# pymoc/pymoc

Measured on AMD Instinct MI355X. Metric: column-timesteps/sec (ensemble) at nz=100, higher is better.
Workload: dtype f64; 1 GPU; BASELINE configs[1]: 1024 independent Columns x nz=100 fp64 per GPU, static wA, do_conv on odd members, dt=30 d (pymoc_amd.configs.config2); columns_per_gpu=1024, nz=100, kernel=k_column_steps<64,2,6,true,true>, parallelism=ensemble sharded over 1 GPU(s), RCCL gather (root) of the final state

## Files before the change

### pymoc_amd/csrc/column.hip.h

```cpp
#pragma once
#include <type_traits>
#include "common.hip.h"

namespace pm {

template <int P>
struct ColGrid {
  double z[P];
  double dz[P];
  double dzc[P];
  double rdz[P], rdzc[P];
  double rdz_l[P], rdzc_l[P];
};
template <int P>
struct ColRegs {
  double b[P];
  double kap[P];
  double area[P];
  double dAk[P];
  double rarea[P];
  double rarea_l[P];
  double area_u, rarea_u, rarea_lu;
};

template <int P>
__device__ __forceinline__ void load_levels(double (&out)[P], const double *__restrict__ row,
                                            int lg, int nz, int lvl0 = 0) {
  if constexpr (P == 2) {
    if (lvl0 == 0 && (nz & 1) == 0 && (((unsigned long long)row) & 15ull) == 0ull) {
      const int i0 = lg * 2 < nz - 2 ? lg * 2 : nz - 2;
      const double2 v = *reinterpret_cast<const double2 *>(row + i0);
      out[0] = v.x;
      out[1] = v.y;
      return;
    }
  }
#pragma unroll
  for (int p = 0; p < P; ++p) {
    const int i = lvl0 + lg * P + p;
    out[p] = row[i < nz ? i : nz - 1];
  }
}

template <int P>
__device__ __forceinline__ double level_value(const double (&x)[P], int j) {
  const int jl = __builtin_amdgcn_readfirstlane(j / P);
  const int jp = __builtin_amdgcn_readfirstlane(j % P);
  double out = 0.;
#pragma unroll
  for (int p = 0; p < P; ++p) {
    const int lo = __builtin_amdgcn_readlane(__double2loint(x[p]), jl);
    const int hi = __builtin_amdgcn_readlane(__double2hiint(x[p]), jl);
    const double v = __hiloint2double(hi, lo);
    out = (p == 0 || jp == p) ? v : out;
  }
  return out;
}

__device__ __forceinline__ double lane_value(double x, int lane) {
  const int lo = __builtin_amdgcn_readlane(__double2loint(x), lane);
  const int hi = __builtin_amdgcn_readlane(__double2hiint(x), lane);
  return __hiloint2double(hi, lo);
}

template <int P>
struct ConvCache {
  unsigned long long mask[P];
  double zconv;
  bool valid = false;
};

template <int G, int P>
__device__ __forceinline__ bool col_convect(double (&b)[P], const double (&z)[P],
                                            double bs, double N2min, int lg, int lane,
                                            int nz, const double *__restrict__ zg,
                                            ConvCache<P> *cache = nullptr) {
  const unsigned long long gm = group_mask<G>(lane);
  bool ind[P];
  unsigned long long im[P];
  unsigned long long anym = 0ull;
#pragma unroll
  for (int p = 0; p < P; ++p) {
    const int i = lg * P + p;
    ind[p] = (i < nz) && (b[p] > bs);
    im[p] = __builtin_amdgcn_ballot_w64(ind[p]);
    anym |= im[p] & gm;
  }
  if (__builtin_expect(anym != 0ull, 0)) {
    double zconv;
    bool hit = false;
    if constexpr (G == 64) {
      if (cache != nullptr && cache->valid) {
        hit = true;
#pragma unroll
        for (int p = 0; p < P; ++p) hit = hit && (cache->mask[p] == im[p]);
      }
    }
    if (hit) {
      zconv = cache->zconv;
    } else {
      int jmax = 0;
#pragma unroll
      for (int p = 0; p < P; ++p) {
        const int i = lg * P + p;
        const unsigned long long m = __builtin_amdgcn_ballot_w64((i < nz) && !ind[p]) & gm;
        if (m != 0ull) {
          const int hl = 63 - __clzll((long long)m);
          const int j = (hl % G) * P + p;
          jmax = j > jmax ? j : jmax;
        }
      }
      if constexpr (G == 64) {
        zconv = level_value<P>(z, jmax);
        if (cache != nullptr) {
#pragma unroll
          for (int p = 0; p < P; ++p) cache->mask[p] = im[p];
          cache->zconv = zconv;
          cache->valid = true;
        }
      } else {
        zconv = zg[jmax];
      }
    }
#pragma unroll
    for (int p = 0; p < P; ++p) {
      const double adj = bs + N2min * (z[p] - zconv);
      b[p] = ind[p] ? adj : b[p];
    }
    return true;
  }
#pragma unroll
  for (int p = 0; p < P; ++p)
    if (lg * P + p == nz - 1) b[p] = bs;
  return false;
}

template <int P>
__device__ __forceinline__ void col_convect_cached(double (&b)[P], const double (&z)[P],
                                                   double bs, double N2min, int lane, int nz,
                                                   ConvCache<P> &cc) {
  bool ind[P];
  unsigned long long im[P], anym = 0ull;
  bool same = cc.valid;
#pragma unroll
  for (int p = 0; p < P; ++p) {
    ind[p] = (lane * P + p < nz) && (b[p] > bs);
    im[p] = __builtin_amdgcn_ballot_w64(ind[p]);
    anym |= im[p];
    same = same && (im[p] == cc.mask[p]);
  }
  if (__builtin_expect(!same, 0)) {
    int jmax = 0;
#pragma unroll
    for (int p = 0; p < P; ++p) {
      const unsigned long long m = __builtin_amdgcn_ballot_w64((lane * P + p < nz) && !ind[p]);
      if (m != 0ull) {
        const int j = (63 - __clzll((long long)m)) * P + p;
        jmax = j > jmax ? j : jmax;
      }
    }
    cc.zconv = level_value<P>(z, jmax);
#pragma unroll
    for (int p = 0; p < P; ++p) cc.mask[p] = im[p];
    cc.valid = true;
  }
  const bool none = anym == 0ull;
#pragma unroll
  for (int p = 0; p < P; ++p) {
    const double adj = bs + N2min * (z[p] - cc.zconv);
    b[p] = ind[p] ? adj : b[p];
    if (lane * P + p == nz - 1) b[p] = none ? bs : b[p];
  }
}

template <int G, int P, int DIV, bool BC = true, bool WEFF = false, bool UA = false,
          bool FLUXFMA = (DIV == 2 || DIV >= 6)>
__device__ __forceinline__ void col_vertadvdiff(const ColGrid<P> &g, ColRegs<P> &r,
                                                const double (&wA)[P],
                                                double dt, bool do_conv, double bs,
                                                double bbot, bool use_bzbot,
                                                double bzbot, int lg, int nz,
                                                int lvl0 = 0) {
  if (BC && !do_conv) {
#pragma unroll
    for (int p = 0; p < P; ++p)
      if (lvl0 + lg * P + p == nz - 1) r.b[p] = bs;
  }
  const double nb0 = from_next_lane_z(r.b[0]);
  double bup[P];
#pragma unroll
  for (int p = 0; p < P; ++p) bup[p] = (p < P - 1) ? r.b[p + 1 < P ? p + 1 : p] : nb0;
  if (BC && lvl0 + lg * P == 0) r.b[0] = use_bzbot ? (bup[0] - bzbot * g.dz[0]) : bbot;

  if constexpr (DIV == 4) {
    double d_up[P];
#pragma unroll
    for (int p = 0; p < P; ++p) d_up[p] = bup[p] - r.b[p];
    const double pd = from_prev_lane_z(d_up[P - 1]);
#pragma unroll
    for (int p = 0; p < P; ++p) {
      const double d_dn = (p > 0) ? d_up[p > 0 ? p - 1 : 0] : pd;
      r.b[p] = __builtin_fma(r.kap[p], d_up[p], __builtin_fma(r.dAk[p], d_dn, r.b[p]));
    }
    return;
  }
  double bz[P];
  {
    double num[P], q[P], rr[P];
#pragma unroll
    for (int p = 0; p < P; ++p) num[p] = bup[p] - r.b[p];
    if constexpr (DIV == 2) {
#pragma unroll
      for (int p = 0; p < P; ++p) rr[p] = num[p] * g.rdz_l[p];
#pragma unroll
      for (int p = 0; p < P; ++p) q[p] = __builtin_fma(num[p], g.rdz[p], rr[p]);
#pragma unroll
      for (int p = 0; p < P; ++p) rr[p] = __builtin_fma(-g.dz[p], q[p], num[p]);
#pragma unroll
      for (int p = 0; p < P; ++p) q[p] = __builtin_fma(rr[p], g.rdz[p], q[p]);
    } else if constexpr (DIV == 7 || DIV == 8) {
#pragma unroll
      for (int p = 0; p < P; ++p) rr[p] = num[p] * g.rdz_l[p];
#pragma unroll
      for (int p = 0; p < P; ++p) q[p] = __builtin_fma(num[p], g.rdz[p], rr[p]);
    } else if constexpr (DIV == 6) {
#pragma unroll
      for (int p = 0; p < P; ++p) q[p] = num[p] * g.rdz[p];
#pragma unroll
      for (int p = 0; p < P; ++p) rr[p] = __builtin_fma(-g.dz[p], q[p], num[p]);
#pragma unroll
      for (int p = 0; p < P; ++p) q[p] = __builtin_fma(rr[p], g.rdz[p], q[p]);
    } else if constexpr (DIV == 1 || DIV == 3 || DIV == 5) {
#pragma unroll
      for (int p = 0; p < P; ++p) q[p] = num[p] * g.rdz[p];
#pragma unroll
      for (int p = 0; p < P; ++p) rr[p] = __builtin_fma(-g.dz[p], q[p], num[p]);
#pragma unroll
      for (int p = 0; p < P; ++p) q[p] = __builtin_fma(rr[p], g.rdz[p], q[p]);
#pragma unroll
      for (int p = 0; p < P; ++p) rr[p] = __builtin_fma(-g.dz[p], q[p], num[p]);
#pragma unroll
      for (int p = 0; p < P; ++p) q[p] = __builtin_fma(rr[p], g.rdz[p], q[p]);
    } else {
#pragma unroll
      for (int p = 0; p < P; ++p) q[p] = num[p] / g.dz[p];
    }
    if constexpr (DIV != 0) {
#pragma unroll
      for (int p = 0; p < P; ++p) bz[p] = q[p];
    } else {
#pragma unroll
      for (int p = 0; p < P; ++p) bz[p] = (lvl0 + lg * P + p < nz - 1) ? q[p] : 0.0;
    }
  }
  const double pbz = from_prev_lane_z(bz[P - 1]);
  double bz_dn[P], dbz[P], flx[P], bzz[P], adv[P];
#pragma unroll
  for (int p = 0; p < P; ++p) {
    bz_dn[p] = (p > 0) ? bz[p > 0 ? p - 1 : 0] : pbz;
    dbz[p] = bz[p] - bz_dn[p];
    const double weff = WEFF ? wA[p] : wA[p] - r.dAk[p];
    if constexpr (FLUXFMA) {
      const double wn = (weff < 0.0) ? -weff : 0.0, wp = (weff < 0.0) ? 0.0 : -weff;
      flx[p] = __builtin_fma(wn, bz[p], wp * bz_dn[p]);
    } else {
      const double bzu = (weff < 0.0) ? bz[p] : bz_dn[p];
      flx[p] = (-weff) * bzu;
    }
  }
  if constexpr (DIV == 2) {
    double r1[P], r2[P];
#pragma unroll
    for (int p = 0; p < P; ++p) {
      r1[p] = dbz[p] * g.rdzc_l[p];
      r2[p] = flx[p] * (UA ? r.rarea_lu : r.rarea_l[p]);
    }
#pragma unroll
    for (int p = 0; p < P; ++p) {
      bzz[p] = __builtin_fma(dbz[p], g.rdzc[p], r1[p]);
      adv[p] = __builtin_fma(flx[p], (UA ? r.rarea_u : r.rarea[p]), r2[p]);
    }
#pragma unroll
    for (int p = 0; p < P; ++p) {
      r1[p] = __builtin_fma(-g.dzc[p], bzz[p], dbz[p]);
      r2[p] = __builtin_fma(-(UA ? r.area_u : r.area[p]), adv[p], flx[p]);
    }
#pragma unroll
    for (int p = 0; p < P; ++p) {
      bzz[p] = __builtin_fma(r1[p], g.rdzc[p], bzz[p]);
      adv[p] = __builtin_fma(r2[p], (UA ? r.rarea_u : r.rarea[p]), adv[p]);
    }
  } else if constexpr (DIV == 6) {
    double r1[P], r2[P];
#pragma unroll
    for (int p = 0; p < P; ++p) {
      bzz[p] = dbz[p] * g.rdzc[p];
      adv[p] = flx[p] * (UA ? r.rarea_u : r.rarea[p]);
    }
#pragma unroll
    for (int p = 0; p < P; ++p) {
      r1[p] = __builtin_fma(-g.dzc[p], bzz[p], dbz[p]);
      r2[p] = __builtin_fma(-(UA ? r.area_u : r.area[p]), adv[p], flx[p]);
    }
#pragma unroll
    for (int p = 0; p < P; ++p) {
      bzz[p] = __builtin_fma(r1[p], g.rdzc[p], bzz[p]);
      adv[p] = __builtin_fma(r2[p], (UA ? r.rarea_u : r.rarea[p]), adv[p]);
    }
  } else if constexpr (DIV == 8) {
    double r1[P], r2[P];
#pragma unroll
    for (int p = 0; p < P; ++p) {
      r1[p] = dbz[p] * g.rdzc_l[p];
      r2[p] = flx[p] * (UA ? r.rarea_lu : r.rarea_l[p]);
    }
#pragma unroll
    for (int p = 0; p < P; ++p) {
      bzz[p] = __builtin_fma(dbz[p], g.rdzc[p], r1[p]);
      adv[p] = __builtin_fma(flx[p], (UA ? r.rarea_u : r.rarea[p]), r2[p]);
    }
  } else if constexpr (DIV == 7) {
    double r1[P], r2[P];
#pragma unroll
    for (int p = 0; p < P; ++p) {
      r1[p] = dbz[p] * g.rdzc_l[p];
      adv[p] = flx[p] * (UA ? r.rarea_u : r.rarea[p]);
    }
#pragma unroll
    for (int p = 0; p < P; ++p) {
      bzz[p] = __builtin_fma(dbz[p], g.rdzc[p], r1[p]);
      r2[p] = __builtin_fma(-(UA ? r.area_u : r.area[p]), adv[p], flx[p]);
    }
#pragma unroll
    for (int p = 0; p < P; ++p) adv[p] = __builtin_fma(r2[p], (UA ? r.rarea_u : r.rarea[p]), adv[p]);
  } else if constexpr (DIV == 5) {
    double r1[P];
#pragma unroll
    for (int p = 0; p < P; ++p) {
      bzz[p] = dbz[p] * g.rdzc[p];
      adv[p] = div_by_recip2(flx[p], r.area_u, r.rarea_u, r.rarea_lu);
    }
#pragma unroll
    for (int k = 0; k < 2; ++k) {
#pragma unroll
      for (int p = 0; p < P; ++p) r1[p] = __builtin_fma(-g.dzc[p], bzz[p], dbz[p]);
#pragma unroll
      for (int p = 0; p < P; ++p) bzz[p] = __builtin_fma(r1[p], g.rdzc[p], bzz[p]);
    }
  } else if constexpr (DIV == 3) {
    double r1[P];
#pragma unroll
    for (int p = 0; p < P; ++p) {
      bzz[p] = dbz[p] * g.rdzc[p];
      adv[p] = flx[p] / (UA ? r.area_u : r.area[p]);
    }
#pragma unroll
    for (int k = 0; k < 2; ++k) {
#pragma unroll
      for (int p = 0; p < P; ++p) r1[p] = __builtin_fma(-g.dzc[p], bzz[p], dbz[p]);
#pragma unroll
      for (int p = 0; p < P; ++p) bzz[p] = __builtin_fma(r1[p], g.rdzc[p], bzz[p]);
    }
  } else if constexpr (DIV == 1) {
    double r1[P], r2[P];
#pragma unroll
    for (int p = 0; p < P; ++p) {
      bzz[p] = dbz[p] * g.rdzc[p];
      adv[p] = flx[p] * (UA ? r.rarea_u : r.rarea[p]);
    }
#pragma unroll
    for (int k = 0; k < 2; ++k) {
#pragma unroll
      for (int p = 0; p < P; ++p) {
        r1[p] = __builtin_fma(-g.dzc[p], bzz[p], dbz[p]);
        r2[p] = __builtin_fma(-(UA ? r.area_u : r.area[p]), adv[p], flx[p]);
      }
#pragma unroll
      for (int p = 0; p < P; ++p) {
        bzz[p] = __builtin_fma(r1[p], g.rdzc[p], bzz[p]);
        adv[p] = __builtin_fma(r2[p], (UA ? r.rarea_u : r.rarea[p]), adv[p]);
      }
    }
  } else {
#pragma unroll
    for (int p = 0; p < P; ++p) {
      bzz[p] = dbz[p] / g.dzc[p];
      adv[p] = flx[p] / (UA ? r.area_u : r.area[p]);
    }
  }
#pragma unroll
  for (int p = 0; p < P; ++p) {
    const int i = lvl0 + lg * P + p;
    const bool interior = (i >= 1) && (i <= nz - 2);
    const double db_dt = adv[p] + r.kap[p] * bzz[p];
    if constexpr (DIV == 0) {
      const double nb = r.b[p] + dt * db_dt;
      r.b[p] = interior ? nb : r.b[p];
    } else {
      r.b[p] = r.b[p] + (interior ? dt : 0.0) * db_dt;
    }
  }
}

template <int P>
__device__ __forceinline__ void col_horadv(ColRegs<P> &r, const double (&vdx)[P],
                                           const double (&bin)[P], double dt, int lg,
                                           int nz) {
#pragma unroll
  for (int p = 0; p < P; ++p) {
    const int i = lg * P + p;
    if (i < nz && vdx[p] > 0.0) {
      const double db = bin[p] - r.b[p];
      r.b[p] = r.b[p] + dt * vdx[p] * db / r.area[p];
    }
  }
}

template <int P>
__device__ __forceinline__ bool col_inputs_in_fast_range(const ColGrid<P> &g, const ColRegs<P> &r,
                                                         const double (&wA)[P], double dt,
                                                         double bs, double bbot, double bzbot,
                                                         double N2min, int lg, int nz) {
  bool ok = in_fast_div_range(dt) && in_fast_div_range(bs) && in_fast_div_range(bbot) &&
            in_fast_div_range(bzbot) && in_fast_div_range(N2min);
#pragma unroll
  for (int p = 0; p < P; ++p) {
    const bool top = lg * P + p >= nz - 1;
    ok = ok && in_fast_div_range(r.b[p]) && in_fast_div_range(wA[p]) &&
         in_fast_div_range(r.dAk[p]) && in_fast_div_range(wA[p] - r.dAk[p]) &&
         in_fast_div_range(r.kap[p]) && in_fast_div_range(r.area[p]) && r.area[p] != 0.0 &&
         in_fast_div_range(g.z[p]) && (top || (in_fast_div_range(g.dz[p]) && g.dz[p] != 0.0)) &&
         in_fast_div_range(g.dzc[p]) && g.dzc[p] != 0.0;
  }
  return ok;
}

template <int P>
__device__ __forceinline__ bool col_state_in_fast_range(const ColRegs<P> &r, const double (&wA)[P]) {
  int ok = 1;
#pragma unroll
  for (int p = 0; p < P; ++p)
    ok &= (int)in_fast_div_range(r.b[p]) & (int)in_fast_div_range(wA[p] - r.dAk[p]);
  return ok != 0;
}

template <int P, int DIV = 1>
__device__ __forceinline__ void col_load_grid(ColGrid<P> &g, const pm_columns &c, int lg,
                                              int lvl0 = 0) {
  const int nz = c.nz;
#pragma unroll
  for (int p = 0; p < P; ++p) {
    const int i = lvl0 + lg * P + p;
    const int ic = i < nz ? i : nz - 1;
    const int iu = ic + 1 < nz ? ic + 1 : nz - 1;
    const int id = ic > 0 ? ic - 1 : 0;
    const double zc = c.z[ic];
    g.z[p] = zc;
    g.dz[p] = c.z[iu] - zc;
    g.dzc[p] = 0.5 * (g.dz[p] + (zc - c.z[id]));
    if constexpr (DIV != 0 && DIV != 4) {
      g.rdz[p] = (i < nz - 1) ? 1.0 / g.dz[p] : 0.0;
      g.rdzc[p] = 1.0 / g.dzc[p];
    } else {
      g.rdz[p] = g.rdzc[p] = 0.0;
    }
    if constexpr (DIV == 2) {
      g.rdz_l[p] = (i < nz - 1) ? recip_lo(g.dz[p], g.rdz[p]) : 0.0;
      g.rdzc_l[p] = recip_lo(g.dzc[p], g.rdzc[p]);
    } else {
      g.rdz_l[p] = g.rdzc_l[p] = 0.0;
    }
  }
}

template <int P, int DIV = 1>
__device__ __forceinline__ void col_load_static(ColRegs<P> &r, const pm_columns &c,
                                                int col, int sel, int lg, int lvl0 = 0,
                                                bool uniform_area = false, bool weff_in = false) {
  const int nz = c.nz;
  const size_t base = (size_t)col * nz;
  const size_t sbase = ((size_t)sel * c.ncols + col) * nz;
  load_levels<P>(r.kap, c.kappa + sbase, lg, nz, lvl0);
  if (!weff_in) {
    load_levels<P>(r.dAk, c.dAkappa + sbase, lg, nz, lvl0);
  } else {
#pragma unroll
    for (int p = 0; p < P; ++p) r.dAk[p] = 0.0;
  }
  if (uniform_area) {
    const double a0 = c.area[base];
    const double ra = (DIV != 0 && DIV != 4) ? 1.0 / a0 : 0.0;
    const double ral = DIV == 2 ? recip_lo(a0, ra) : 0.0;
#pragma unroll
    for (int p = 0; p < P; ++p) {
      r.area[p] = a0;
      r.rarea[p] = ra;
      r.rarea_l[p] = ral;
    }
    return;
  }
  load_levels<P>(r.area, c.area + base, lg, nz, lvl0);
#pragma unroll
  for (int p = 0; p < P; ++p) {
    r.rarea[p] = (DIV != 0 && DIV != 4) ? 1.0 / r.area[p] : 0.0;
    r.rarea_l[p] = DIV == 2 ? recip_lo(r.area[p], r.rarea[p]) : 0.0;
  }
}

template <int P>
__device__ __forceinline__ void col_make_contracted(const ColGrid<P> &g, ColRegs<P> &r,
                                                    const double (&wA)[P], double dt, int lane,
                                                    int nz) {
  const double dz_prev_lane = from_prev_lane_z(g.dz[P - 1]);
#pragma unroll
  for (int p = 0; p < P; ++p) {
    const int i = lane * P + p;
    const bool interior = i >= 1 && i <= nz - 2;
    const double weff = wA[p] - r.dAk[p];
    const double dz_up = interior ? g.dz[p] : 1.0;
    const double dz_dn = interior ? ((p > 0) ? g.dz[p > 0 ? p - 1 : 0] : dz_prev_lane) : 1.0;
    const double dzc = interior ? g.dzc[p] : 1.0, area = interior ? r.area[p] : 1.0;
    const double wn = (weff < 0.0) ? -weff : 0.0, wp = (weff < 0.0) ? 0.0 : -weff;
    const double cu = dt * (r.kap[p] / (dzc * dz_up) + wn / (area * dz_up));
    const double cl = dt * (-r.kap[p] / (dzc * dz_dn) + wp / (area * dz_dn));
    r.kap[p] = interior ? cu : 0.0;
    r.dAk[p] = interior ? cl : 0.0;
  }
}

template <int P>
__device__ __forceinline__ unsigned conv_variant(const ConvCache<P> &cc) {
  unsigned need = 0u;
#pragma unroll
  for (int p = 0; p < P; ++p) need |= (cc.mask[p] != 0ull) ? (1u << p) : 0u;
  if constexpr (P <= 2) {
    return need;
  } else {
    return need ? (1u << P) - 1u : 0u;
  }
}

template <int P, int DIV, unsigned SEL, bool UA = false>
__device__ __forceinline__ int conv_spec_run(const ColGrid<P> &g, ColRegs<P> &r,
                                             const double (&wA)[P], double dt, double bs,
                                             double bbot, double N2min, int lane, int nz,
                                             ConvCache<P> &cc, int s, int nsteps) {
  constexpr int UNR = P <= 2 ? 16 : (P <= 4 ? 2 : 1);
  double adjv[P];
  double bs_eff[P];
  auto set_adj = [&]() {
#pragma unroll
    for (int p = 0; p < P; ++p)
      adjv[p] = (lane * P + p == 0) ? bbot : bs + N2min * (g.z[p] - cc.zconv);
  };
  set_adj();
#pragma unroll
  for (int p = 0; p < P; ++p) bs_eff[p] = (lane * P + p < nz) ? bs : __builtin_inf();
  double b_blk[P];
  unsigned long long acc;
  double bmax[P];
  auto spec = [&]() {
    unsigned long long im[P];
    bool ind[P];
#pragma unroll
    for (int p = 0; p < P; ++p) {
      if (((SEL >> p) & 1u) != 0u) {
        ind[p] = r.b[p] > bs_eff[p];
        im[p] = __builtin_amdgcn_ballot_w64(ind[p]);
      } else {
        bmax[p] = __builtin_fmax(bmax[p], r.b[p]);
      }
    }
#pragma unroll
    for (int p = 0; p < P; ++p) {
      if (((SEL >> p) & 1u) != 0u) r.b[p] = ind[p] ? adjv[p] : r.b[p];
    }
    col_vertadvdiff<64, P, DIV, false, false, UA>(g, r, wA, dt, true, bs, bbot, false, 0., lane, nz);
#pragma unroll
    for (int p = 0; p < P; ++p) {
      if (((SEL >> p) & 1u) != 0u) {
        unsigned long long x;
        asm("s_xor_b64 %0, %1, %2" : "=s"(x) : "s"(im[p]), "s"(cc.mask[p]) : "scc");
        acc |= x;
      }
    }
  };
  auto block_begin = [&]() {
    acc = 0ull;
#pragma unroll
    for (int p = 0; p < P; ++p) {
      b_blk[p] = r.b[p];
      bmax[p] = -__builtin_inf();
    }
  };
  auto block_bad = [&]() -> bool {
    bool conv = false;
#pragma unroll
    for (int p = 0; p < P; ++p)
      if (((SEL >> p) & 1u) == 0u) conv = conv || (bmax[p] > bs_eff[p]);
    if constexpr (SEL != (1u << P) - 1u) {
      unsigned long long any = __builtin_amdgcn_ballot_w64(conv);
      asm("" : "+s"(any));
      acc |= any;
    }
    return acc != 0ull;
  };
  auto redo = [&](int nb) {
#pragma unroll
    for (int p = 0; p < P; ++p) r.b[p] = b_blk[p];
    for (int k = 0; k < nb; ++k) {
      col_convect_cached<P>(r.b, g.z, bs, N2min, lane, nz, cc);
      if (lane == 0) r.b[0] = bbot;
      col_vertadvdiff<64, P, DIV, false, false, UA>(g, r, wA, dt, true, bs, bbot, false, 0., lane, nz);
    }
  };
  int pos = s, ret = -1;
  auto tier = [&](auto U) {
    constexpr int N = decltype(U)::value;
    int left = (nsteps - pos) / N;
    const int s_end = pos + left * N;
    for (; left > 0; --left) {
      block_begin();
#pragma unroll
      for (int k = 0; k < N; ++k) spec();
      if (__builtin_expect(block_bad(), 0)) {
        redo(N);
        if (conv_variant<P>(cc) != SEL) {
          ret = s_end - (left - 1) * N;
          left = 1;
        } else {
          set_adj();
        }
      }
    }
    pos = s_end;
  };
  if (UNR <= 4 || nsteps - pos >= 4 * UNR) tier(std::integral_constant<int, UNR>{});
  if (ret >= 0) return ret;
  if constexpr (UNR > 4) {
    tier(std::integral_constant<int, 4>{});
    if (ret >= 0) return ret;
  }
  if constexpr (UNR > 1) tier(std::integral_constant<int, 1>{});
  return ret >= 0 ? ret : nsteps;
}

template <int G, int P>
__device__ __forceinline__ void col_store_result(const pm_columns &c, const ColRegs<P> &r,
                                                 size_t base, int col, bool col_ok, int lg,
                                                 int lane, int nz) {
  bool bad = false;
  bool stored = false;
  if constexpr (P == 2) {
    if ((nz & 1) == 0 && (((unsigned long long)(c.b + base)) & 15ull) == 0ull) {
      if (lg * 2 < nz) {
        if (col_ok) *reinterpret_cast<double2 *>(c.b + base + lg * 2) = make_double2(r.b[0], r.b[1]);
        bad = !isfinite(r.b[0]) || !isfinite(r.b[1]);
      }
      stored = true;
    }
  }
  if (!stored) {
#pragma unroll
    for (int p = 0; p < P; ++p) {
      const int i = lg * P + p;
      if (i < nz) {
        if (col_ok) c.b[base + i] = r.b[p];
        bad |= !isfinite(r.b[p]);
      }
    }
  }
  if (c.nonfinite) {
    const unsigned long long m = __ballot(bad) & group_mask<G>(lane);
    if (lg == 0 && col_ok) c.nonfinite[col] = (m != 0ull) ? 1 : 0;
  }
}

template <int P>
__device__ __forceinline__ void col_pin(double (&b)[P]) {
#pragma unroll
  for (int p = 0; p < P; ++p) asm volatile("" : "+v"(b[p]));
}

template <int G, int P, int FAST, bool PLAIN, bool UA = false>
__global__ __launch_bounds__(256) void k_column_steps(
    pm_columns c, const double *__restrict__ wA_g, const double *__restrict__ vdx_g,
    const double *__restrict__ bin_g, double dt, int nsteps, int ops) {
  const int lane = threadIdx.x & (WAVE - 1);
  const int lg = threadIdx.x % G;
  int col_raw = (int)((blockIdx.x * (unsigned)blockDim.x + threadIdx.x) / G);
  constexpr bool FORMS = FAST == 6 && G == 64 && P <= 2 && PLAIN;
  if constexpr (FORMS) col_raw = __builtin_amdgcn_readfirstlane(col_raw);
  const bool col_ok = col_raw < c.ncols;
  const int col = col_ok ? col_raw : c.ncols - 1;
  const int nz = c.nz;
  const size_t base = (size_t)col * nz;

  ColGrid<P> g;
  ColRegs<P> r;
  const int sel = c.ksel ? c.ksel[col] : 0;
  const int flags = c.flags ? c.flags[col] : 0;
  col_load_grid<P, FAST>(g, c, lg);
  const bool ua = G == 64 && __builtin_amdgcn_readfirstlane(flags & PM_COL_UNIFORM_AREA) != 0;
  col_load_static<P, FAST>(r, c, col, sel, lg, 0, ua, (ops & PM_OP_WEFF) != 0);
  if constexpr (UA) {
    r.area_u = lane_value(r.area[0], 0);
    r.rarea_u = lane_value(r.rarea[0], 0);
    r.rarea_lu = lane_value(r.rarea_l[0], 0);
  }

  double wA[P], vdx[P], bin[P];
  load_levels<P>(r.b, c.b + base, lg, nz);
#pragma unroll
  for (int p = 0; p < P; ++p) wA[p] = vdx[p] = bin[p] = 0.0;
  const bool wA_row = !(PLAIN && (ops & PM_OP_WA_TWOBASIN) != 0 && col >= 2 * (c.ncols / 3));
  if (wA_g && wA_row) load_levels<P>(wA, wA_g + base, lg, nz);
  if constexpr (PLAIN) {
    if (ops & PM_OP_WA_PSI) {
      const int half = c.ncols >> 1;
      if (col < half) {
        if (bin_g) {
          double pso[P];
          load_levels<P>(pso, bin_g + base, lg, nz);
#pragma unroll
          for (int p = 0; p < P; ++p) wA[p] = (wA[p] - pso[p]) * 1e6;
        } else {
#pragma unroll
          for (int p = 0; p < P; ++p) wA[p] = wA[p] * 1e6;
        }
      } else {
#pragma unroll
        for (int p = 0; p < P; ++p) wA[p] = (-wA[p]) * 1e6;
      }
    }
  }
  if constexpr (PLAIN) {
    if (ops & PM_OP_WA_TWOBASIN) {
      const int third = c.ncols / 3;
      if (col < third) {
        double zon[P], pso[P];
        load_levels<P>(zon, vdx_g + base, lg, nz);
        load_levels<P>(pso, bin_g + base, lg, nz);
#pragma unroll
        for (int p = 0; p < P; ++p) wA[p] = (wA[p] + zon[p] - pso[p]) * 1e6;
      } else if (col < 2 * third) {
#pragma unroll
        for (int p = 0; p < P; ++p) wA[p] = (-wA[p]) * 1e6;
      } else {
        const size_t bp = (size_t)(col - third) * nz;
        double zon[P], pso[P];
        load_levels<P>(zon, vdx_g + bp, lg, nz);
        load_levels<P>(pso, bin_g + bp, lg, nz);
#pragma unroll
        for (int p = 0; p < P; ++p) wA[p] = (-zon[p] - pso[p]) * 1e6;
      }
    }
  }
  const bool wa_formed = (ops & (PM_OP_WA_PSI | PM_OP_WA_TWOBASIN)) != 0;
  if (vdx_g && !wa_formed) load_levels<P>(vdx, vdx_g + base, lg, nz);
  if (bin_g && !wa_formed) load_levels<P>(bin, bin_g + base, lg, nz);
  const bool do_conv = (flags & PM_COL_DO_CONV) != 0;
  const bool use_bzbot = (flags & PM_COL_BZBOT) != 0 && c.bzbot != nullptr;
  const double bs = c.bs[col];
  const double bbot = c.bbot[col];
  const double bzbot = use_bzbot ? c.bzbot[col] : 0.0;
  const double N2min = c.N2min[col];

  if constexpr (FAST != 0) {
    const bool vouched = G == 64 &&
                         __builtin_amdgcn_readfirstlane(flags & PM_COL_STATIC_IN_RANGE) != 0 &&
                         in_fast_div_range(dt);
    bool fast_ok;
    if (vouched)
      fast_ok = col_state_in_fast_range<P>(r, wA);
    else
      fast_ok = col_inputs_in_fast_range<P>(g, r, wA, dt, bs, bbot, bzbot, N2min, lg, nz);
    if (__builtin_expect(__ballot(!fast_ok) != 0ull, 0)) {
      for (int s = 0; s < nsteps; ++s) {
        if ((ops & PM_OP_CONVECT) && do_conv)
          col_convect<G, P>(r.b, g.z, bs, N2min, lg, lane, nz, c.z);
        col_pin<P>(r.b);
        if (ops & PM_OP_VERTADVDIFF)
          col_vertadvdiff<G, P, 0>(g, r, wA, dt, do_conv, bs, bbot, use_bzbot, bzbot, lg, nz);
        if ((ops & PM_OP_HORADV) && vdx_g) col_horadv<P>(r, vdx, bin, dt, lg, nz);
      }
      col_store_result<G, P>(c, r, base, col, col_ok, lg, lane, nz);
      return;
    }
  }

  if constexpr (FAST == 4) col_make_contracted<P>(g, r, wA, dt, lane, nz);

  auto plain_run = [&](auto DIVC) {
    constexpr int DIV = decltype(DIVC)::value;
    if (do_conv && use_bzbot) {
      for (int s = 0; s < nsteps; ++s) {
        col_convect<G, P>(r.b, g.z, bs, N2min, lg, lane, nz, c.z);
        col_vertadvdiff<G, P, DIV, true, false, UA>(g, r, wA, dt, true, bs, bbot, true, bzbot, lg, nz);
      }
    } else if (do_conv) {
      ConvCache<P> cc;
#pragma unroll
      for (int p = 0; p < P; ++p) cc.mask[p] = 0ull;
      cc.zconv = 0.;
      if constexpr (G == 64) {
        col_convect_cached<P>(r.b, g.z, bs, N2min, lane, nz, cc);
        if (lg == 0) r.b[0] = bbot;
        col_vertadvdiff<G, P, DIV, false, false, UA>(g, r, wA, dt, true, bs, bbot, false, 0., lg, nz);
        int s = 1;
        while (s < nsteps) {
          const unsigned v = conv_variant<P>(cc);
          if constexpr (P <= 2) {
            switch (v) {
              case 0: s = conv_spec_run<P, DIV, 0u, UA>(g, r, wA, dt, bs, bbot, N2min, lane, nz, cc, s, nsteps); break;
              case 1: s = conv_spec_run<P, DIV, 1u, UA>(g, r, wA, dt, bs, bbot, N2min, lane, nz, cc, s, nsteps); break;
              case 2: s = conv_spec_run<P, DIV, 2u, UA>(g, r, wA, dt, bs, bbot, N2min, lane, nz, cc, s, nsteps); break;
              default: s = conv_spec_run<P, DIV, 3u, UA>(g, r, wA, dt, bs, bbot, N2min, lane, nz, cc, s, nsteps); break;
            }
          } else {
            if (v == 0u)
              s = conv_spec_run<P, DIV, 0u, UA>(g, r, wA, dt, bs, bbot, N2min, lane, nz, cc, s, nsteps);
            else
              s = conv_spec_run<P, DIV, (1u << P) - 1u, UA>(g, r, wA, dt, bs, bbot, N2min, lane, nz, cc, s, nsteps);
          }
        }
      } else {
        for (int s = 0; s < nsteps; ++s) {
          col_convect<G, P>(r.b, g.z, bs, N2min, lg, lane, nz, c.z);
          if (lg == 0) r.b[0] = bbot;
          col_vertadvdiff<G, P, DIV, false, false, UA>(g, r, wA, dt, true, bs, bbot, false, 0., lg, nz);
        }
      }
    } else if (use_bzbot) {
      for (int s = 0; s < nsteps; ++s)
        col_vertadvdiff<G, P, DIV, true, false, UA>(g, r, wA, dt, false, bs, bbot, true, bzbot, lg, nz);
    } else {
#pragma unroll
      for (int p = 0; p < P; ++p) {
        if (lg * P + p == nz - 1) r.b[p] = bs;
        if (lg * P + p == 0) r.b[p] = bbot;
      }
      int s = 0;
      if constexpr (P <= 2) {
        for (; s + 4 <= nsteps; s += 4) {
          col_vertadvdiff<G, P, DIV, false, false, UA>(g, r, wA, dt, false, bs, bbot, false, 0., lg, nz);
          col_vertadvdiff<G, P, DIV, false, false, UA>(g, r, wA, dt, false, bs, bbot, false, 0., lg, nz);
          col_vertadvdiff<G, P, DIV, false, false, UA>(g, r, wA, dt, false, bs, bbot, false, 0., lg, nz);
          col_vertadvdiff<G, P, DIV, false, false, UA>(g, r, wA, dt, false, bs, bbot, false, 0., lg, nz);
        }
      }
      for (; s < nsteps; ++s)
        col_vertadvdiff<G, P, DIV, false, false, UA>(g, r, wA, dt, false, bs, bbot, false, 0., lg, nz);
    }
  };
  if constexpr (PLAIN) {
    if constexpr (FORMS) {
      const bool d2g = (c.reserved & PM_COLS_DIV3_PROVEN) != 0 && (c.reserved & PM_COLS_DIV2_GRID) != 0;
      if (d2g) {
#pragma unroll
        for (int p = 0; p < P; ++p) {
          const bool below_top = lg * P + p < nz - 1;
          g.rdz_l[p] = below_top ? recip_lo_div(g.dz[p], g.rdz[p]) : 0.0;
          g.rdzc_l[p] = below_top ? recip_lo_div(g.dzc[p], g.rdzc[p]) : 0.0;
        }
        if (__builtin_amdgcn_readfirstlane(flags & PM_COL_DIV2_AREA) != 0) {
          if constexpr (UA) {
            r.rarea_lu = lane_value(recip_lo_div(r.area_u, r.rarea_u), 0);
          } else {
#pragma unroll
            for (int p = 0; p < P; ++p) r.rarea_l[p] = recip_lo_div(r.area[p], r.rarea[p]);
          }
          plain_run(std::integral_constant<int, 8>{});
        } else {
          plain_run(std::integral_constant<int, 7>{});
        }
      } else {
        plain_run(std::integral_constant<int, 6>{});
      }
    } else {
      plain_run(std::integral_constant<int, FAST>{});
    }
  } else {
    for (int s = 0; s < nsteps; ++s) {
      if ((ops & PM_OP_CONVECT) && do_conv)
        col_convect<G, P>(r.b, g.z, bs, N2min, lg, lane, nz, c.z);
      col_pin<P>(r.b);
      if (ops & PM_OP_VERTADVDIFF)
        col_vertadvdiff<G, P, FAST, true, false, UA>(g, r, wA, dt, do_conv, bs, bbot, use_bzbot, bzbot, lg, nz);
      if ((ops & PM_OP_HORADV) && vdx_g) col_horadv<P>(r, vdx, bin, dt, lg, nz);
    }
  }

  col_store_result<G, P>(c, r, base, col, col_ok, lg, lane, nz);
}

template <int P>
struct ColStage {
  double b[P], wA[P], kap[P], area[P], dAk[P];
};
template <int P>
struct ColStageLean {
  double b[P], wA[P];
};

struct StreamScalars {
  int flags, sel;
  double bs, bbot, bzbot, N2min, area0, kbase;
  double ra, ral;
  __device__ __forceinline__ void load(const pm_columns &c, int col0, int cend, int lane) {
    const int col = col0 + lane < cend ? col0 + lane : cend - 1;
    flags = c.flags ? c.flags[col] : 0;
    sel = c.ksel ? c.ksel[col] : 0;
    bs = c.bs[col];
    bbot = c.bbot[col];
    N2min = c.N2min[col];
    bzbot = ((flags & PM_COL_BZBOT) != 0 && c.bzbot != nullptr) ? c.bzbot[col] : 0.0;
    area0 = (flags & PM_COL_UNIFORM_AREA) ? c.area[(size_t)col * c.nz] : 0.0;
    kbase = c.kappa_base ? c.kappa_base[col] : 0.0;
    ra = 1.0 / area0;
    ral = recip_lo(area0, ra);
  }
};

template <int P, bool AFF = false>
__device__ __forceinline__ void col_stage_load(ColStage<P> &s, const pm_columns &c,
                                               const double *__restrict__ wA_g, int col,
                                               int lane, bool weff_in, int flags, int sel,
                                               double area0) {
  const int nz = c.nz;
  const size_t base = (size_t)col * nz;
  const size_t sbase = ((size_t)sel * c.ncols + col) * nz;
  load_levels<P>(s.b, c.b + base, lane, nz);
  load_levels<P>(s.wA, wA_g + base, lane, nz);
  if constexpr (!AFF) load_levels<P>(s.kap, c.kappa + sbase, lane, nz);
  if ((flags & PM_COL_UNIFORM_AREA) == 0) {
    load_levels<P>(s.area, c.area + base, lane, nz);
  } else {
#pragma unroll
    for (int p = 0; p < P; ++p) s.area[p] = area0;
  }
  if (!weff_in) {
    load_levels<P>(s.dAk, c.dAkappa + sbase, lane, nz);
  } else {
#pragma unroll
    for (int p = 0; p < P; ++p) s.dAk[p] = 0.0;
  }
}

template <int P, int D, bool AFF = false, bool LEAN = false, bool VEC = false, bool D3 = false,
          int CPWU = 0, int WEFFT = -1, int UABT = -1>
__global__ __launch_bounds__(256) __attribute__((amdgpu_waves_per_eu((LEAN && P <= 2 && D <= 5) ? 4 : 1)))
void k_column_stream(pm_columns c,
                                                       const double *__restrict__ wA_g,
                                                       double dt, int nsteps, int cpw, bool dt_ok,
                                                       bool weff_in) {
  const int lane = threadIdx.x & (WAVE - 1);
  const int wave = (int)((blockIdx.x * (unsigned)blockDim.x + threadIdx.x) >> 6);
  const int col0 = __builtin_amdgcn_readfirstlane(wave * cpw);
  const int nz = c.nz;
  if (col0 >= c.ncols) return;
  const int cend = col0 + cpw < c.ncols ? col0 + cpw : c.ncols;

  StreamScalars sc;
  sc.load(c, col0, cend, lane);
  static_assert(!LEAN || AFF, "the lean ring needs the affine kappa");
  static_assert(!VEC || (LEAN && P == 2), "16-byte accesses: the lean form with two levels per lane");
  const int off2 = lane * 2 < nz - 2 ? lane * 2 : nz - 2;
  using Stage = typename std::conditional<LEAN, ColStageLean<P>, ColStage<P>>::type;
  auto flags_of = [&](int k) { return __builtin_amdgcn_readlane(sc.flags, k); };
  auto issue = [&](Stage &st, int col) {
    const int k = col - col0;
    if constexpr (VEC) {
      const size_t base = (size_t)col * nz;
      const double2 vb = *reinterpret_cast<const double2 *>(c.b + base + off2);
      const double2 vw = *reinterpret_cast<const double2 *>(wA_g + base + off2);
      st.b[0] = vb.x;
      st.b[P - 1] = vb.y;
      st.wA[0] = vw.x;
      st.wA[P - 1] = vw.y;
    } else if constexpr (LEAN) {
      const size_t base = (size_t)col * nz;
      load_levels<P>(st.b, c.b + base, lane, nz);
      load_levels<P>(st.wA, wA_g + base, lane, nz);
    } else if constexpr (CPWU > 0 && WEFFT >= 0 && UABT >= 0) {
      const int sel = __builtin_amdgcn_readlane(sc.sel, k);
      const size_t base = (size_t)col * nz, sbase = ((size_t)sel * c.ncols + col) * nz;
      load_levels<P>(st.b, c.b + base, lane, nz);
      load_levels<P>(st.wA, wA_g + base, lane, nz);
      if constexpr (!AFF) load_levels<P>(st.kap, c.kappa + sbase, lane, nz);
      if constexpr (UABT == 0) load_levels<P>(st.area, c.area + base, lane, nz);
      if constexpr (WEFFT == 0) load_levels<P>(st.dAk, c.dAkappa + sbase, lane, nz);
    } else {
      col_stage_load<P, AFF>(st, c, wA_g, col, lane, weff_in, flags_of(k),
                             __builtin_amdgcn_readlane(sc.sel, k), lane_value(sc.area0, k));
    }
  };
  ColGrid<P> g;
  col_load_grid<P, 1>(g, c, lane);
  double kprof[P];
#pragma unroll
  for (int p = 0; p < P; ++p) kprof[p] = 0.0;
  if constexpr (AFF) load_levels<P>(kprof, c.kappa_profile, lane, nz);
  Stage ring[D];
#pragma unroll
  for (int d = 0; d < D; ++d)
    if (col0 + d < cend) issue(ring[d], col0 + d);
  unsigned nf_bits = 0u;
  auto one_column = [&](int col, int d, bool prefetch, int kk) {
      ColRegs<P> r;
      double wA[P];
#pragma unroll
      for (int p = 0; p < P; ++p) {
        r.b[p] = ring[d].b[p];
        wA[p] = ring[d].wA[p];
        if constexpr (AFF)
          r.kap[p] = lane_value(sc.kbase, col - col0) + kprof[p];
        else
          r.kap[p] = ring[d].kap[p];
        if constexpr (LEAN) {
          r.area[p] = lane_value(sc.area0, col - col0);
          r.area_u = r.area[p];
          r.rarea_u = lane_value(sc.ra, col - col0);
          r.rarea_lu = lane_value(sc.ral, col - col0);
          r.dAk[p] = 0.0;
        } else if constexpr (CPWU > 0 && WEFFT >= 0 && UABT >= 0) {
          if constexpr (UABT == 1)
            r.area[p] = lane_value(sc.area0, col - col0);
          else
            r.area[p] = ring[d].area[p];
          if constexpr (WEFFT == 1)
            r.dAk[p] = 0.0;
          else
            r.dAk[p] = ring[d].dAk[p];
        } else {
          r.area[p] = ring[d].area[p];
          r.dAk[p] = ring[d].dAk[p];
        }
        r.rarea[p] = r.rarea_l[p] = 0.;
      }
      if (CPWU > 0) {
        if (prefetch) issue(ring[d], col + D);
      } else {
        issue(ring[d], col + D < cend ? col + D : cend - 1);
      }
      const int k = col - col0;
      const int flags = flags_of(k);
      const bool do_conv = (flags & PM_COL_DO_CONV) != 0;
      const bool use_bzbot = (flags & PM_COL_BZBOT) != 0 && c.bzbot != nullptr;
      const double bs = lane_value(sc.bs, k), bbot = lane_value(sc.bbot, k),
                   N2min = lane_value(sc.N2min, k), bzbot = lane_value(sc.bzbot, k);
      const bool fast_ok = ((flags & PM_COL_STATIC_IN_RANGE) != 0 && dt_ok)
                               ? col_state_in_fast_range<P>(r, wA)
                               : col_inputs_in_fast_range<P>(g, r, wA, dt, bs, bbot, bzbot, N2min,
                                                             lane, nz);
      const bool slow = __ballot(!fast_ok) != 0ull;
      for (int s = 0; s < nsteps; ++s) {
        if (do_conv) col_convect<64, P>(r.b, g.z, bs, N2min, lane, lane, nz, c.z);
        col_pin<P>(r.b);
        if (__builtin_expect(slow, 0))
          col_vertadvdiff<64, P, 0>(g, r, wA, dt, do_conv, bs, bbot, use_bzbot, bzbot, lane, nz);
        else if constexpr (LEAN && D3)
          col_vertadvdiff<64, P, 6, true, false, true, false>(g, r, wA, dt, do_conv, bs, bbot, use_bzbot,
                                                              bzbot, lane, nz);
        else if constexpr (LEAN)
          col_vertadvdiff<64, P, 5, true, false, true>(g, r, wA, dt, do_conv, bs, bbot, use_bzbot,
                                                       bzbot, lane, nz);
        else
          col_vertadvdiff<64, P, 3>(g, r, wA, dt, do_conv, bs, bbot, use_bzbot, bzbot, lane, nz);
      }
      const size_t base = (size_t)col * nz;
      bool bad = false;
      bool stored = false;
      if constexpr (VEC) {
        if (lane * 2 < nz) {
          *reinterpret_cast<double2 *>(c.b + base + lane * 2) = make_double2(r.b[0], r.b[P - 1]);
          bad = !isfinite(r.b[0]) || !isfinite(r.b[P - 1]);
        }
        stored = true;
      } else if constexpr (P == 2) {
        if ((nz & 1) == 0 && (((unsigned long long)(c.b + base)) & 15ull) == 0ull) {
          if (lane * 2 < nz) {
            *reinterpret_cast<double2 *>(c.b + base + lane * 2) = make_double2(r.b[0], r.b[1]);
            bad = !isfinite(r.b[0]) || !isfinite(r.b[1]);
          }
          stored = true;
        }
      }
      if (!stored) {
#pragma unroll
        for (int p = 0; p < P; ++p) {
          const int i = lane * P + p;
          if (i < nz) {
            c.b[base + i] = r.b[p];
            bad |= !isfinite(r.b[p]);
          }
        }
      }
      if (CPWU > 0) {
        nf_bits |= (__ballot(bad) != 0ull ? 1u : 0u) << kk;
      } else if (c.nonfinite) {
        const unsigned long long m = __ballot(bad);
        if (lane == 0) c.nonfinite[col] = (m != 0ull) ? 1 : 0;
      }
  };
  if constexpr (CPWU > 0) {
#pragma unroll
    for (int k = 0; k < CPWU; ++k) one_column(col0 + k, k % D, k + D < CPWU, k);
    if (c.nonfinite && lane < CPWU) c.nonfinite[col0 + lane] = (int)((nf_bits >> lane) & 1u);
  } else {
    for (int colb = col0; colb < cend; colb += D) {
#pragma unroll
      for (int d = 0; d < D; ++d) {
        const int col = colb + d;
        if (col >= cend) break;
        one_column(col, d, true, 0);
      }
    }
  }
}

inline int stream_cols_per_wave(int ncols) {
  const int waves_wanted = 1024 * 8;
  int cpw = ncols / waves_wanted;
  return cpw < 1 ? 1 : (cpw > 32 ? 32 : cpw);
}

inline int pick_levels_per_lane(int G, int need) {
  static const int sup64[] = {1, 2, 3, 4, 5, 6, 7, 8, 10, 13, 16};
  static const int sup[] = {1, 2, 3, 4, 5, 6, 7, 8};
  if (G == 64) {
    for (int v : sup64)
      if (v >= need) return v;
  } else {
    for (int v : sup)
      if (v >= need) return v;
  }
  return -1;
}

struct ColKernel {
  bool stream, plain, ua, aff, lean, vec, d3;
  int fast, d, cpwu, wefft, uabt;
  constexpr bool compiled(int G, int P) const {
    if (!stream && !ua && fast <= 2) return true;
    return G == 64 && P <= 4 && (P == 2 || (!vec && cpwu == 0));
  }
};
constexpr ColKernel col_steps(int fast, bool plain, bool ua = false) {
  return {false, plain, ua, false, false, false, false, fast, 0, 0, -1, -1};
}
constexpr ColKernel col_stream(int d, bool aff = false, bool lean = false, bool vec = false,
                               bool d3 = false, int cpwu = 0, int wefft = -1, int uabt = -1) {
  return {true, false, false, aff, lean, vec, d3, 0, d, cpwu, wefft, uabt};
}

#define PM_COLUMN_KERNELS(X)                                                                   \
  X(CK_STEPS_IEEE, col_steps(0, false))                                         \
  X(CK_STEPS_RECIP, col_steps(1, false))              \
  X(CK_STEPS_PLAIN, col_steps(2, true))                              \
  X(CK_STEPS_PLAIN_UA, col_steps(2, true, true))                \
  X(CK_STEPS_DIV3_UA, col_steps(6, true, true))           \
  X(CK_STEPS_CONTRACTED, col_steps(4, true))                         \
  X(CK_STREAM, col_stream(2))                                \
  X(CK_STREAM_WEFF, col_stream(3))                                    \
  X(CK_STREAM_AFF, col_stream(3, true))                 \
  X(CK_STREAM_WEFF_AFF, col_stream(4, true))                                                   \
  X(CK_STREAM_LEAN, col_stream(5, true, true))            \
  X(CK_STREAM_LEAN_VEC, col_stream(5, true, true, true))             \
  X(CK_STREAM_LEAN_VEC_D3, col_stream(5, true, true, true, true))                              \
  X(CK_STREAM_LEAN_VEC_U8, col_stream(5, true, true, true, false, 8))       \
  X(CK_STREAM_LEAN_VEC_D3_U8, col_stream(5, true, true, true, true, 8))                        \
  X(CK_STREAM_U8, col_stream(2, false, false, false, false, 8, 0, 0))                          \
  X(CK_STREAM_WEFF_UA_U8, col_stream(3, false, false, false, false, 8, 1, 1))

#define PM_CK_ID(id, args) id,
enum ColKernelId { CK_NONE, PM_COLUMN_KERNELS(PM_CK_ID) };
#undef PM_CK_ID
constexpr ColKernel col_kernel(ColKernelId k) {
#define PM_CK_ARGS(id, args) \
  case id: return args;
  switch (k) {
    PM_COLUMN_KERNELS(PM_CK_ARGS)
    default: return {};
  }
#undef PM_CK_ARGS
}

struct ColumnPlan {
  ColKernelId kernel;
  int G, P;
  int cpw;
  unsigned grid;
};

inline ColumnPlan column_plan(const pm_columns &c, const double *wA, const double *vdx, int nsteps,
                              int ops, int G, int P) {
  const bool weff = (ops & PM_OP_WEFF) != 0;
  const bool plain =
      (ops & ~(PM_OP_WEFF | PM_OP_CONTRACTED | PM_OP_WA_PSI | PM_OP_WA_TWOBASIN)) == PM_OP_TIMESTEP &&
      (!vdx || (ops & PM_OP_WA_TWOBASIN));
  const bool ua = (c.reserved & PM_COLS_ALL_UNIFORM_AREA) != 0;
  const bool d3 = (c.reserved & PM_COLS_DIV3_PROVEN) != 0;
  const bool aff = c.kappa_base && c.kappa_profile && c.nsel == 1;
  const bool wave_per_col = G == 64 && P <= 4;
  const int cpw = stream_cols_per_wave(c.ncols);
  ColumnPlan pl{CK_STEPS_IEEE, G, P, 0, (unsigned)((c.ncols + 256 / G - 1) / (256 / G))};
  if (wave_per_col && nsteps < 3 && plain && cpw >= 2) {
    pl.cpw = cpw;
    if (weff && aff && ua) {
      pl.cpw = c.ncols / 16384 < 2 ? 2 : (c.ncols / 16384 > 16 ? 16 : c.ncols / 16384);
      const bool vec = P == 2 && (c.nz & 1) == 0 &&
                       ((((unsigned long long)c.b) | ((unsigned long long)wA)) & 15ull) == 0ull;
      const bool u8 = vec && c.ncols % 8 == 0 && c.ncols >= 8 * 4096;
      if (u8) pl.cpw = 8;
      pl.kernel = !vec ? CK_STREAM_LEAN
                  : u8 ? (d3 ? CK_STREAM_LEAN_VEC_D3_U8 : CK_STREAM_LEAN_VEC_U8)
                       : (d3 ? CK_STREAM_LEAN_VEC_D3 : CK_STREAM_LEAN_VEC);
    } else if (P == 2 && !aff && c.ncols % 8 == 0 && c.ncols >= 8 * 4096 && weff == ua) {
      pl.cpw = 8;
      pl.kernel = weff ? CK_STREAM_WEFF_UA_U8 : CK_STREAM_U8;
    } else {
      pl.kernel = weff ? (aff ? CK_STREAM_WEFF_AFF : CK_STREAM_WEFF) : (aff ? CK_STREAM_AFF : CK_STREAM);
    }
    const unsigned waves = (unsigned)((c.ncols + pl.cpw - 1) / pl.cpw);
    pl.grid = (waves + 3) / 4;
  } else if (nsteps >= 3 && plain) {
    if (wave_per_col && (ops & PM_OP_CONTRACTED))
      pl.kernel = CK_STEPS_CONTRACTED;
    else if (wave_per_col && ua)
      pl.kernel = d3 ? CK_STEPS_DIV3_UA : CK_STEPS_PLAIN_UA;
    else
      pl.kernel = CK_STEPS_PLAIN;
  } else if (nsteps >= 3) {
    pl.kernel = CK_STEPS_RECIP;
  }
  return pl;
}

inline int column_kernel_name(const ColumnPlan &pl, char *name, size_t len) {
  const ColKernel k = col_kernel(pl.kernel);
  auto tf = [](bool v) { return v ? "true" : "false"; };
  int n = 0;
  if (pl.kernel == CK_NONE)
    n = snprintf(name, len, "%s", "");
  else if (k.stream)
    n = snprintf(name, len, "k_column_stream<%d,%d,%s,%s,%s,%s,%d,%d,%d>", pl.P, k.d, tf(k.aff),
                 tf(k.lean), tf(k.vec), tf(k.d3), k.cpwu, k.wefft, k.uabt);
  else
    n = snprintf(name, len, "k_column_steps<%d,%d,%d,%s,%s>", pl.G, pl.P, k.fast, tf(k.plain),
                 tf(k.ua));
  PM_REQUIRE(n >= 0 && (size_t)n < len, "name buffer of %zu bytes too small", len);
  return PM_OK;
}

template <int G, int P, ColKernelId K>
int launch_column_kernel(const ColumnPlan &pl, const pm_columns &c, const double *wA,
                         const double *vdx, const double *bin, double dt, int nsteps, int ops,
                         hipStream_t st) {
  constexpr ColKernel k = col_kernel(K);
  if constexpr (!k.compiled(G, P)) {
    return fail(PM_EINVAL, "column kernel %d is not compiled for G=%d P=%d", (int)K, G, P);
  } else if constexpr (k.stream) {
    const double adt = dt < 0 ? -dt : dt;
    const bool dt_ok = dt == 0.0 || (adt >= 0x1p-200 && adt <= 0x1p200);
    hipLaunchKernelGGL((k_column_stream<P, k.d, k.aff, k.lean, k.vec, k.d3, k.cpwu, k.wefft, k.uabt>),
                       dim3(pl.grid), dim3(256), 0, st, c, wA, dt, nsteps, pl.cpw, dt_ok,
                       (ops & PM_OP_WEFF) != 0);
  } else {
    hipLaunchKernelGGL((k_column_steps<G, P, k.fast, k.plain, k.ua>), dim3(pl.grid), dim3(256), 0,
                       st, c, wA, vdx, bin, dt, nsteps, ops & ~PM_OP_CONTRACTED);
  }
  PM_HIP(hipGetLastError());
  return PM_OK;
}

template <int G, int P>
int launch_column_steps(const ColumnPlan &pl, const pm_columns &c, const double *wA,
                        const double *vdx, const double *bin, double dt, int nsteps, int ops,
                        hipStream_t st) {
#define PM_CK_LAUNCH(id, args) \
  case id: return launch_column_kernel<G, P, id>(pl, c, wA, vdx, bin, dt, nsteps, ops, st);
  switch (pl.kernel) {
    PM_COLUMN_KERNELS(PM_CK_LAUNCH)
    default: return PM_OK;
  }
#undef PM_CK_LAUNCH
}

int column_steps_g16(const ColumnPlan &pl, const pm_columns &c, const double *wA,
                     const double *vdx, const double *bin, double dt, int nsteps, int ops,
                     hipStream_t st);
int column_steps_g32(const ColumnPlan &pl, const pm_columns &c, const double *wA,
                     const double *vdx, const double *bin, double dt, int nsteps, int ops,
                     hipStream_t st);
int column_steps_g64(const ColumnPlan &pl, const pm_columns &c, const double *wA,
                     const double *vdx, const double *bin, double dt, int nsteps, int ops,
                     hipStream_t st);
int column_steps_implicit(const pm_columns &c, const double *wA, const double *zon,
                          const double *so, double dt, int nsteps, int ops, hipStream_t st);

}
```

Before: 13.81 billion column-timesteps/s.

## Hold surface-level convection bit so speculative no-convection variant stays selected

Adds a 'held' flag to the convection cache that marks when the only convecting level is the surface cell, whose value stays above bs. That bit is then excluded from variant selection and from the speculative block-validity ballot, so columns whose surface sits above bs can run the cheaper SEL variant instead of the full-convection path. A NaN check is added to the validity test so that excluding the held bit cannot hide a diverging state. It also adds a probe script for per-wave lifetimes. The risk is that if the held surface case does not stay stable, blocks get redone more often.

```diff
diff --git a/profiles/r07/probe_wave_classes.py b/profiles/r07/probe_wave_classes.py
--- /dev/null
+++ b/profiles/r07/probe_wave_classes.py
@@ -0,0 +1,80 @@
+import ctypes as C
+import os
+import sys
+
+sys.path.insert(0, os.path.dirname(os.path.dirname(os.path.dirname(os.path.abspath(__file__)))))
+import numpy as np
+import pymoc_amd as gpu
+from pymoc_amd import configs, _lib
+from pymoc_amd.device import DeviceArray
+
+N, F = 1024, 1000
+LABEL = os.environ.get("LABEL", "tree")
+ROUNDS = int(os.environ.get("ROUNDS", 5))
+
+c = configs.config2(N=N)
+batch = gpu.ColumnBatch(c["z"], c["kappa"], c["Area"], c["b0"], bs=c["bs"], bbot=c["bbot"],
+                        N2min=c["N2min"], do_conv=c["do_conv"])
+wA = DeviceArray.from_host(c["wA"])
+flagged = np.asarray(c["do_conv"], dtype=bool)
+form8 = np.asarray(batch.div2_area_proven, dtype=bool)
+surface = flagged & (c["b0"][:, -1] > c["bs"])
+classes = [
+    ("not flagged, form 8", ~flagged & form8),
+    ("not flagged, form 7", ~flagged & ~form8),
+    ("flagged, surface at bs, form 8", flagged & ~surface & form8),
+    ("flagged, surface at bs, form 7", flagged & ~surface & ~form8),
+    ("flagged, surface above bs, form 8", flagged & surface & form8),
+    ("flagged, surface above bs, form 7", flagged & surface & ~form8),
+]
+
+for _ in range(3):
+  batch.steps(wA, c["dt"], F)
+gpu.synchronize()
+
+lines = ["## %s: `%s`" % (LABEL, batch.kernel_name(F)), ""]
+stamps = (C.c_ulonglong * (3 * N))()
+life_all = []
+for rnd in range(ROUNDS):
+  batch.steps(wA, c["dt"], F)
+  gpu.synchronize()
+  if _lib.lib.pm_debug_col_stamps(stamps, N) != 0:
+    raise SystemExit("pm_debug_col_stamps failed")
+  s = np.array(list(stamps), dtype=np.uint64).reshape(N, 3)
+  t0, t1, cls = s[:, 0].astype(np.int64), s[:, 1].astype(np.int64), s[:, 2].astype(np.int64)
+  life_all.append((t1 - t0).astype(np.float64))
+life = np.median(np.array(life_all), axis=0)
+order = np.argsort(-life)
+
+lines += ["One wave per column; lifetime = last stamp - first stamp in shader cycles, per wave the median "
+          "over %d launches of 1000 steps (after 3 warm-up launches)." % ROUNDS, "",
+          "| class | columns | step form / last SEL seen by the kernel | median lifetime | max lifetime | median / class 3 |",
+          "|---|---|---|---|---|---|"]
+ref = np.median(life[classes[2][1]])
+for name, m in classes:
+  if not m.any():
+    lines.append("| %s | 0 | - | - | - | - |" % name)
+    continue
+  seen = sorted(set("%d/%s" % (v >> 8, "plain" if (v & 0xff) == 0xff else str(v & 0xff)) for v in cls[m].tolist()))
+  lines.append("| %s | %d | %s | %.0f | %.0f | %.4f |" % (name, int(m.sum()), ", ".join(seen),
+               np.median(life[m]), life[m].max(), np.median(life[m]) / ref))
+names = np.empty(N, dtype=object)
+for name, m in classes:
+  names[m] = name
+lines += ["", "Longest-lived 8 waves: " + "; ".join(
+    "col %d (%s) %.0f" % (int(i), names[i], life[i]) for i in order[:8])]
+top = order[:int(surface.sum())]
+lines += ["", "Of the %d longest-lived waves, %d are of the class 'flagged, surface above bs'." %
+          (top.size, int(surface[top].sum()))]
+nxt = order[int(surface.sum()):][:4]
+lines += ["The next 4: " + "; ".join("col %d (%s) %.0f" % (int(i), names[i], life[i]) for i in nxt)]
+lines += ["Per-launch variation of a wave's lifetime (max - min over the launches), median over waves: %.0f cycles." %
+          float(np.median(np.ptp(np.array(life_all), axis=0)))]
+text = "\n".join(lines) + "\n"
+print(text)
+out = os.environ.get("OUT")
+if out:
+  os.makedirs(out, exist_ok=True)
+  with open(os.path.join(out, "r07_wave_classes_%s.md" % LABEL), "w") as f:
+    f.write(text)
+  np.save(os.path.join(out, "r07_wave_life_%s.npy" % LABEL), np.array(life_all))
diff --git a/pymoc_amd/csrc/column.hip.h b/pymoc_amd/csrc/column.hip.h
--- a/pymoc_amd/csrc/column.hip.h
+++ b/pymoc_amd/csrc/column.hip.h
@@ -68,6 +68,7 @@
   unsigned long long mask[P];
   double zconv;
   bool valid = false;
+  bool held = false;
 };
 
 template <int G, int P>
@@ -529,15 +530,34 @@
 }
 
 template <int P>
-__device__ __forceinline__ unsigned conv_variant(const ConvCache<P> &cc) {
+__device__ __forceinline__ unsigned long long conv_held_bit(const ConvCache<P> &cc, int p, int nz) {
+  const int sl = (nz - 1) / P, sp = (nz - 1) - sl * P;
+  return (cc.held && p == sp) ? 1ull << sl : 0ull;
+}
+
+template <int P>
+__device__ __forceinline__ unsigned conv_variant(const ConvCache<P> &cc, int nz) {
   unsigned need = 0u;
 #pragma unroll
-  for (int p = 0; p < P; ++p) need |= (cc.mask[p] != 0ull) ? (1u << p) : 0u;
+  for (int p = 0; p < P; ++p)
+    need |= ((cc.mask[p] & ~conv_held_bit<P>(cc, p, nz)) != 0ull) ? (1u << p) : 0u;
   if constexpr (P <= 2) {
     return need;
   } else {
     return need ? (1u << P) - 1u : 0u;
   }
+}
+
+template <int P>
+__device__ __forceinline__ void conv_hold_surface(ConvCache<P> &cc, const double (&b)[P],
+                                                  const double (&z)[P], double bs, double N2min,
+                                                  int lane, int nz) {
+  const int sl = (nz - 1) / P, sp = (nz - 1) - sl * P;
+  unsigned long long m = 0ull;
+#pragma unroll
+  for (int p = 0; p < P; ++p) m = (p == sp) ? cc.mask[p] : m;
+  const double v = level_value<P>(b, nz - 1);
+  cc.held = __builtin_amdgcn_ballot_w64(((m >> sl) & 1ull) != 0ull && v > bs && v != 0.0) != 0ull;
 }
 
 template <int P, int DIV, unsigned SEL, bool UA = false>
@@ -548,10 +568,13 @@
   constexpr int UNR = P <= 2 ? 16 : (P <= 4 ? 2 : 1);
   double adjv[P];
   double bs_eff[P];
+  unsigned long long hb[P];
   auto set_adj = [&]() {
 #pragma unroll
-    for (int p = 0; p < P; ++p)
+    for (int p = 0; p < P; ++p) {
       adjv[p] = (lane * P + p == 0) ? bbot : bs + N2min * (g.z[p] - cc.zconv);
+      hb[p] = conv_held_bit<P>(cc, p, nz);
+    }
   };
   set_adj();
 #pragma unroll
@@ -594,12 +617,20 @@
     }
   };
   auto block_bad = [&]() -> bool {
-    bool conv = false;
-#pragma unroll
-    for (int p = 0; p < P; ++p)
-      if (((SEL >> p) & 1u) == 0u) conv = conv || (bmax[p] > bs_eff[p]);
     if constexpr (SEL != (1u << P) - 1u) {
-      unsigned long long any = __builtin_amdgcn_ballot_w64(conv);
+      unsigned long long any = 0ull;
+      bool un = false;
+#pragma unroll
+      for (int p = 0; p < P; ++p)
+        if (((SEL >> p) & 1u) == 0u) any |= __builtin_amdgcn_ballot_w64(bmax[p] > bs_eff[p]) & ~hb[p];
+#pragma unroll
+      for (int p = 0; p < P; p += 2) {
+        const bool a = ((SEL >> p) & 1u) == 0u, b = p + 1 < P && ((SEL >> (p + 1)) & 1u) == 0u;
+        if (a && b) un = un || __builtin_isunordered(r.b[p], r.b[p + 1 < P ? p + 1 : p]);
+        else if (a) un = un || __builtin_isunordered(r.b[p], r.b[p]);
+        else if (b) un = un || __builtin_isunordered(r.b[p + 1 < P ? p + 1 : p], r.b[p + 1 < P ? p + 1 : p]);
+      }
+      any |= __builtin_amdgcn_ballot_w64(un);
       asm("" : "+s"(any));
       acc |= any;
     }
@@ -613,6 +644,7 @@
       if (lane == 0) r.b[0] = bbot;
       col_vertadvdiff<64, P, DIV, false, false, UA>(g, r, wA, dt, true, bs, bbot, false, 0., lane, nz);
     }
+    conv_hold_surface<P>(cc, r.b, g.z, bs, N2min, lane, nz);
   };
   int pos = s, ret = -1;
   auto tier = [&](auto U) {
@@ -625,7 +657,7 @@
       for (int k = 0; k < N; ++k) spec();
       if (__builtin_expect(block_bad(), 0)) {
         redo(N);
-        if (conv_variant<P>(cc) != SEL) {
+        if (conv_variant<P>(cc, nz) != SEL) {
           ret = s_end - (left - 1) * N;
           left = 1;
         } else {
@@ -807,9 +839,10 @@
         col_convect_cached<P>(r.b, g.z, bs, N2min, lane, nz, cc);
         if (lg == 0) r.b[0] = bbot;
         col_vertadvdiff<G, P, DIV, false, false, UA>(g, r, wA, dt, true, bs, bbot, false, 0., lg, nz);
+        conv_hold_surface<P>(cc, r.b, g.z, bs, N2min, lane, nz);
         int s = 1;
         while (s < nsteps) {
-          const unsigned v = conv_variant<P>(cc);
+          const unsigned v = conv_variant<P>(cc, nz);
           if constexpr (P <= 2) {
             switch (v) {
               case 0: s = conv_spec_run<P, DIV, 0u, UA>(g, r, wA, dt, bs, bbot, N2min, lane, nz, cc, s, nsteps); break;
```

Result: no change. 13.90 billion column-timesteps/s (median of 6 runs) (+0.6%).
